# m96-chan/PyGPUkit

Measured on AMD Instinct MI355X. Metric: decode tokens/sec/GPU + prefill TFLOPS (% MFMA peak), Qwen3-0.6B bf16, higher is better.
Workload: dtype bf16

## Files before the change

pygpukit_amd/csrc/engine_attn.hip.h:

```cpp
#pragma once

#include "attn_core.hip.h"
#include "engine_state.hip.h"

namespace pgk {

struct AttnArgs {
    const float* qkv;
    int qkv_ld;
    const bf16 *q_gamma, *k_gamma;
    float eps;
    const float *rope_cos, *rope_sin;
    bf16 *kcache, *vcache;
    const int32_t* positions;
    int hq, hkv, max_seq;
    int span;
    float scale;
    float* part;
    int nsplit;
    float* attn_direct;
    const bf16* w_o;
    const bf16* w_o_scale;
    int H, rows_per_block;
    float* opart;
    bf16* attn_direct16;
    int g_total, g_off;
};

template <int D, int G>
struct NewToken {
    float qf[G][8], kn[8], vn[8];
    uint4 qb[G], kbits, vbits;
};

template <int G>
struct NewTokenRaw {
    float4 lo[G + 2], hi[G + 2];
    uint4 gq, gk;
    float4 cs[2], sn[2];
};

template <int D, int G>
__device__ __forceinline__ void new_token_load(const AttnArgs& a, int b, int kvh, int lane, NewTokenRaw<G>& r) {
    constexpr int LPR = D / 8, HALF = D / 2;
    const int sub = lane % LPR;
    const float* row = a.qkv + (size_t)b * a.qkv_ld;
#pragma unroll
    for (int g = 0; g < G + 2; ++g) {
        const unsigned eoff = (g < G) ? (unsigned)(kvh * a.g_total + a.g_off + g) * D : (g == G ? (unsigned)(a.hq + kvh) * D : (unsigned)(a.hq + a.hkv + kvh) * D);
        r.lo[g] = *reinterpret_cast<const float4*>(row + eoff + sub * 8);
        r.hi[g] = *reinterpret_cast<const float4*>(row + eoff + sub * 8 + 4);
    }
    r.gq = r.gk = make_uint4(0, 0, 0, 0);
    if (a.q_gamma != nullptr) {
        r.gq = *reinterpret_cast<const uint4*>(a.q_gamma + sub * 8);
        r.gk = *reinterpret_cast<const uint4*>(a.k_gamma + sub * 8);
    }
    const int dd = (sub * 8) % HALF;
    const float* cs = a.rope_cos + (size_t)b * HALF + dd;
    const float* sn = a.rope_sin + (size_t)b * HALF + dd;
    r.cs[0] = *reinterpret_cast<const float4*>(cs); r.cs[1] = *reinterpret_cast<const float4*>(cs + 4);
    r.sn[0] = *reinterpret_cast<const float4*>(sn); r.sn[1] = *reinterpret_cast<const float4*>(sn + 4);
}

template <int D, int G>
__device__ __forceinline__ void new_token_finish(const AttnArgs& a, int lane, const NewTokenRaw<G>& r, NewToken<D, G>& t) {
    constexpr int LPR = D / 8;
    const int sub = lane % LPR;
    float raw[G + 2][8], gq[8], gk[8];
#pragma unroll
    for (int g = 0; g < G + 2; ++g) {
        raw[g][0] = r.lo[g].x; raw[g][1] = r.lo[g].y; raw[g][2] = r.lo[g].z; raw[g][3] = r.lo[g].w;
        raw[g][4] = r.hi[g].x; raw[g][5] = r.hi[g].y; raw[g][6] = r.hi[g].z; raw[g][7] = r.hi[g].w;
    }
    const bool has_norm = a.q_gamma != nullptr;
    if (has_norm) {
        WTraits<bf16>::decode(r.gq, gq);
        WTraits<bf16>::decode(r.gk, gk);
    } else {
#pragma unroll
        for (int j = 0; j < 8; ++j) gq[j] = gk[j] = 1.f;
    }
    const float csv[8] = {r.cs[0].x, r.cs[0].y, r.cs[0].z, r.cs[0].w, r.cs[1].x, r.cs[1].y, r.cs[1].z, r.cs[1].w};
    const float snv[8] = {r.sn[0].x, r.sn[0].y, r.sn[0].z, r.sn[0].w, r.sn[1].x, r.sn[1].y, r.sn[1].z, r.sn[1].w};
    auto norm_rope = [&](const float (&xin)[8], const float (&gamma)[8], float (&o)[8]) {
        float x[8];
#pragma unroll
        for (int j = 0; j < 8; ++j) x[j] = xin[j];
        if (has_norm) {
            float ss = 0.f;
#pragma unroll
            for (int j = 0; j < 8; ++j) ss = fmaf(x[j], x[j], ss);
            ss = group_sum<LPR>(ss);
            const float inv = 1.0f / sqrtf(ss / D + a.eps);
#pragma unroll
            for (int j = 0; j < 8; ++j) x[j] = x[j] * inv * gamma[j];
        }
        const bool lo = sub < LPR / 2;
#pragma unroll
        for (int j = 0; j < 8; ++j) {
            const float other = xor_half<LPR>(x[j]);
            o[j] = lo ? (x[j] * csv[j] - other * snv[j]) : (x[j] * csv[j] + other * snv[j]);
        }
    };
#pragma unroll
    for (int g = 0; g < G; ++g) {
        norm_rope(raw[g], gq, t.qf[g]);
#pragma unroll
        for (int j = 0; j < 8; ++j) t.qf[g][j] *= a.scale;
        Vec<bf16> qv;
        qv.from_float(t.qf[g]);
        qv.to_float(t.qf[g]);
        t.qb[g] = qv.raw;
    }
    norm_rope(raw[G], gk, t.kn);
#pragma unroll
    for (int j = 0; j < 8; ++j) t.vn[j] = raw[G + 1][j];
    Vec<bf16> kb, vb;
    kb.from_float(t.kn);
    vb.from_float(t.vn);
    kb.to_float(t.kn);
    vb.to_float(t.vn);
    t.kbits = kb.raw;
    t.vbits = vb.raw;
}

template <int D, int G>
__device__ __forceinline__ void prepare_new_token(const AttnArgs& a, int b, int kvh, int pos, int lane, NewToken<D, G>& t) {
    NewTokenRaw<G> r;
    new_token_load<D, G>(a, b, kvh, lane, r);
    new_token_finish<D, G>(a, lane, r, t);
}

template <int D, int G>
__device__ __forceinline__ void fold_new_token(const NewToken<D, G>& t, DecodeState<G>& st) {
    constexpr int LPR = D / 8;
    float s[G];
#pragma unroll
    for (int g = 0; g < G; ++g) {
        float dsum = 0.f;
#pragma unroll
        for (int j = 0; j < 8; ++j) dsum = fmaf(t.qf[g][j], t.kn[j], dsum);
        dsum = group_sum<LPR>(dsum);
        s[g] = dsum;
    }
    st.update(s, t.vn);
}

template <int D, int G, bool DIRECT>
__global__ __launch_bounds__(256) void attn_decode_kernel(unsigned long long* tl, AttnArgs a) {
    const TLStamp tls(tl);
    constexpr int LPR = D / 8, PPW = 64 / LPR, RS = D + 2;
    __shared__ __attribute__((aligned(16))) float lds[4 * PPW * G * RS];
    __shared__ float attn_out[DIRECT ? G * D : 1];
    const int lane = threadIdx.x & 63, wid = threadIdx.x >> 6, sub = lane % LPR;
    const int kvh = blockIdx.y, b = blockIdx.z;
    const size_t head_off = (((size_t)b * a.hkv + kvh) * a.max_seq) * D;
    if constexpr (DIRECT) {
        constexpr int U0 = 8, UB = 4;
        NewTokenRaw<G> raw;
        new_token_load<D, G>(a, b, kvh, lane, raw);
        __builtin_amdgcn_sched_barrier(0);
        KVBatch<U0> kb0;
        kv_issue<D, U0, 4>(kb0, a.kcache + head_off, a.vcache + head_off, wid * PPW, a.max_seq - 1, lane);
        __builtin_amdgcn_sched_barrier(0);
        const int pos = load_uniform_i32(a.positions + b);
        const int c1 = min(pos, a.max_seq);
        KVBatch<UB> kb1;
        kv_issue<D, UB, 4>(kb1, a.kcache + head_off, a.vcache + head_off, U0 * 4 * PPW + wid * PPW, max(c1 - 1, 0), lane);
        __builtin_amdgcn_sched_barrier(0);
        NewToken<D, G> t;
        new_token_finish<D, G>(a, lane, raw, t);
        if (pos < a.max_seq && wid == 0 && lane < LPR && a.g_off == 0) {
            *reinterpret_cast<uint4*>(a.kcache + head_off + (size_t)pos * D + sub * 8) = t.kbits;
            *reinterpret_cast<uint4*>(a.vcache + head_off + (size_t)pos * D + sub * 8) = t.vbits;
        }
        DecodeState<G> st;
        st.init();
        kv_consume<D, G, U0, 4>(kb0, wid * PPW, c1, t.qb, lane, st);
        kv_consume<D, G, UB, 4>(kb1, U0 * 4 * PPW + wid * PPW, c1, t.qb, lane, st);
        if (c1 > (U0 + UB) * 4 * PPW) decode_walk_trips<D, G>(a.kcache + head_off, a.vcache + head_off, (U0 + UB) * 4 * PPW, c1, t.qb, lane, wid, st);
        if (pos < a.max_seq && wid == 0 && lane < LPR) fold_new_token<D, G>(t, st);
        decode_block_merge_lds<D, G>(st, lds, attn_out, lane, wid);
        if (a.attn_direct16) {
            for (int e = threadIdx.x; e < G * D; e += 256) a.attn_direct16[((size_t)b * a.hq + (size_t)kvh * a.g_total + a.g_off) * D + e] = from_f<bf16>(attn_out[e]);
        } else {
            for (int e = threadIdx.x; e < G * D; e += 256) a.attn_direct[((size_t)b * a.hq + (size_t)kvh * a.g_total + a.g_off) * D + e] = attn_out[e];
        }
        tls.end();
        return;
    }
    constexpr int U1 = 8;
    const int chunk = decode_chunk_len(a.span, a.nsplit, 4 * PPW);
    const int c0 = (int)blockIdx.x * chunk;
    NewTokenRaw<G> raw;
    new_token_load<D, G>(a, b, kvh, lane, raw);
    __builtin_amdgcn_sched_barrier(0);
    KVBatch<U1> kb0;
    kv_issue<D, U1, 4>(kb0, a.kcache + head_off, a.vcache + head_off, c0 + wid * PPW, a.max_seq - 1, lane);
    __builtin_amdgcn_sched_barrier(0);
    const int pos = load_uniform_i32(a.positions + b);
    const int ctx = min(pos + 1, a.max_seq);
    tls.phase(0);
    NewToken<D, G> t;
    new_token_finish<D, G>(a, lane, raw, t);
    tls.phase(1);
    const bool last_slice = (int)blockIdx.x == a.nsplit - 1;
    const int c1 = last_slice ? ctx : min(c0 + chunk, ctx);
    const bool owns_new = (pos < a.max_seq) && (pos >= c0) && (last_slice || pos < c0 + chunk);
    if (owns_new && wid == 0 && lane < LPR && a.g_off == 0) {
        *reinterpret_cast<uint4*>(a.kcache + head_off + (size_t)pos * D + sub * 8) = t.kbits;
        *reinterpret_cast<uint4*>(a.vcache + head_off + (size_t)pos * D + sub * 8) = t.vbits;
    }
    DecodeState<G> st;
    st.init();
    const int cend = owns_new ? min(c1, pos) : c1;
    kv_consume<D, G, U1, 4>(kb0, c0 + wid * PPW, cend, t.qb, lane, st);
    if (cend > c0 + U1 * 4 * PPW)
        decode_walk_trips<D, G>(a.kcache + head_off, a.vcache + head_off, c0 + U1 * 4 * PPW, cend, t.qb, lane, wid, st);
    if (owns_new && wid == 0 && lane < LPR) fold_new_token<D, G>(t, st);
    tls.phase(2);
    if constexpr (DIRECT) {
        decode_block_merge_lds<D, G>(st, lds, attn_out, lane, wid);
        for (int e = threadIdx.x; e < G * D; e += 256) a.attn_direct[((size_t)b * a.hq + (size_t)kvh * a.g_total + a.g_off) * D + e] = attn_out[e];
    } else {
        decode_block_merge<D, G>(st, lds, a.part + (((size_t)b * a.hq + (size_t)kvh * a.g_total + a.g_off) * a.nsplit + blockIdx.x) * RS,
                                 (size_t)a.nsplit * RS, lane, wid);
    }
    tls.end();
}

template <int D>
__global__ void attn_merge_kernel(unsigned long long* tl, const float* part, float* attn, int hq, int nsplit) {
    const TLStamp tls(tl);
    __shared__ float w_s[64];
    __shared__ float inv_l;
    const int h = blockIdx.x, b = blockIdx.y, d = threadIdx.x;
    const float* recs = part + ((size_t)b * hq + h) * nsplit * (D + 2);
    if (threadIdx.x < 64) {
        const int s = threadIdx.x;
        const int sc = min(s, nsplit - 1);
        float m = recs[(size_t)sc * (D + 2)], l = recs[(size_t)sc * (D + 2) + 1];
        if (s >= nsplit) { m = -INFINITY; l = 0.f; }
        const float mx = wave_max(m);
        const float w = (m == -INFINITY) ? 0.f : __expf(m - mx);
        const float tot = wave_sum(w * l);
        w_s[s] = w;
        if (s == 0) inv_l = tot > 0.f ? 1.0f / tot : 0.f;
    }
    __syncthreads();
    float o = 0.f;
    int s = 0;
    for (; s + 8 <= nsplit; s += 8) {
        float v[8];
#pragma unroll
        for (int u = 0; u < 8; ++u) v[u] = recs[(size_t)(s + u) * (D + 2) + 2 + d];
#pragma unroll
        for (int u = 0; u < 8; ++u) o = fmaf(w_s[s + u], v[u], o);
    }
    for (; s < nsplit; ++s) o = fmaf(w_s[s], recs[(size_t)s * (D + 2) + 2 + d], o);
    attn[((size_t)b * hq + h) * D + d] = o * inv_l;
    tls.end();
}

template <int D, int G>
__global__ __launch_bounds__(256) void attn_oproj_kernel(unsigned long long* tl, AttnArgs a) {
    const TLStamp tls(tl);
#ifdef PGK_PHASE_STAMPS
    if (threadIdx.x == 0) g_phase_tl = tl;
    __syncthreads();
#endif
    constexpr int NWV = 4;
    constexpr int LPR = D / 8, PPW = 64 / LPR, RS = D + 2;
    constexpr int GD = G * D, LPW = GD / 8;
    constexpr int RPP = NWV * 64 / LPW;
    constexpr int PRE = 4;
    constexpr int U0 = 12;
    __shared__ __attribute__((aligned(16))) float lds[NWV * PPW * G * RS];
    __shared__ __attribute__((aligned(16))) float attn[GD];
    const int lane = threadIdx.x & 63, wid = __builtin_amdgcn_readfirstlane(threadIdx.x >> 6), sub = lane % LPR;
    const int kvh = blockIdx.x % a.hkv, rb = blockIdx.x / a.hkv, b = blockIdx.z;
    const int r0 = rb * a.rows_per_block;
    const int lr = threadIdx.x % LPW, rip = threadIdx.x / LPW;
    const int npass = a.rows_per_block / RPP;
    const bf16* wbase = a.w_o + (size_t)kvh * GD + lr * 8;
    const int ldw = a.hq * D;
    const size_t head_off = (((size_t)b * a.hkv + kvh) * a.max_seq) * D;
    uint4 pre[PRE];
    KVBatch<U0> kb0;
    NewTokenRaw<G> raw;
    new_token_load<D, G>(a, b, kvh, lane, raw);
    __builtin_amdgcn_sched_barrier(0);
    kv_issue<D, U0, NWV>(kb0, a.kcache + head_off, a.vcache + head_off, wid * PPW, a.max_seq - 1, lane);
#pragma unroll
    for (int p = 0; p < PRE; ++p)
        pre[p] = load_nt16(wbase + (size_t)(r0 + min(p, npass - 1) * RPP + rip) * ldw);
    __builtin_amdgcn_sched_barrier(0);
    const int pos = load_uniform_i32(a.positions + b);
    tls.phase(0);
    NewToken<D, G> t;
    new_token_finish<D, G>(a, lane, raw, t);
    if (rb == 0 && pos < a.max_seq && wid == 0 && lane < LPR) {
        *reinterpret_cast<uint4*>(a.kcache + head_off + (size_t)pos * D + sub * 8) = t.kbits;
        *reinterpret_cast<uint4*>(a.vcache + head_off + (size_t)pos * D + sub * 8) = t.vbits;
    }
    tls.phase(1);
    DecodeState<G> st;
    st.init();
    const int c1 = min(pos, a.max_seq);
    kv_consume<D, G, U0, NWV>(kb0, wid * PPW, c1, t.qb, lane, st);
    if (c1 > U0 * NWV * PPW)
        decode_walk_trips<D, G, 8, NWV>(a.kcache + head_off, a.vcache + head_off, U0 * NWV * PPW, c1, t.qb, lane, wid, st);
    if (wid == 0 && lane < LPR) fold_new_token<D, G>(t, st);
    tls.phase(2);
    decode_block_merge_lds<D, G, NWV>(st, lds, attn, lane, wid);
    tls.phase(3);

    float xf[8];
    {
        const float4 u = *reinterpret_cast<const float4*>(attn + lr * 8), v = *reinterpret_cast<const float4*>(attn + lr * 8 + 4);
        xf[0] = u.x; xf[1] = u.y; xf[2] = u.z; xf[3] = u.w; xf[4] = v.x; xf[5] = v.y; xf[6] = v.z; xf[7] = v.w;
    }
    float* outp = a.opart + ((size_t)b * a.hkv + kvh) * a.H;
    for (int p = 0; p < npass; ++p) {
        const int row = r0 + p * RPP + rip;
        uint4 w = (p < PRE) ? pre[p < PRE ? p : 0] : load_nt16(wbase + (size_t)row * ldw);
        float wf[8];
        WTraits<bf16>::decode(w, wf);
        float acc = 0.f;
#pragma unroll
        for (int j = 0; j < 8; ++j) acc = fmaf(wf[j], xf[j], acc);
        acc = group_sum<LPW>(acc);
        if (lr == 0) outp[row] = acc;
    }
    tls.phase(4);
    tls.end();
}

constexpr int AM_CHUNK = 192;

__device__ __forceinline__ int am_koff(int row, int ch) { return row * 256 + ((ch ^ (row & 15)) << 4); }
__device__ __forceinline__ int am_voff(int row, int ch) { return row * 256 + ((ch ^ (((row & 3) << 2) | ((row >> 2) & 3))) << 4); }

template <int G, bool OPROJ = true>
__global__ __launch_bounds__(256) void attn_oproj_mfma_kernel(unsigned long long* tl, AttnArgs a) {
    const TLStamp tls(tl);
    typedef __bf16 am_bf16x8 __attribute__((ext_vector_type(8)));
    typedef float am_f32x4 __attribute__((ext_vector_type(4)));
    typedef short am_v4s __attribute__((ext_vector_type(4)));
    constexpr int D = 128, NWV = 4, LPR = 16, RS = D + 4;
    constexpr int GD = G * D, LPW = GD / 8, RPP = NWV * 64 / LPW, PRE = OPROJ ? 4 : 0;
    extern __shared__ __attribute__((aligned(16))) char am_lds[];
    char* k_lds = am_lds;
    char* v_lds = am_lds + AM_CHUNK * 256;
    __shared__ __attribute__((aligned(16))) float part[NWV + 1][G][RS];
    __shared__ __attribute__((aligned(16))) float attn[GD];
    const int lane = threadIdx.x & 63, wid = __builtin_amdgcn_readfirstlane(threadIdx.x >> 6);
    const int l15 = lane & 15, q4 = lane >> 4;
    const int kvh = blockIdx.x % a.hkv, rb = blockIdx.x / a.hkv, b = blockIdx.z;
    const int r0 = rb * a.rows_per_block;
    const int lr = threadIdx.x % LPW, rip = threadIdx.x / LPW;
    const int npass = a.rows_per_block / RPP;
    const bf16* wbase = a.w_o + (size_t)kvh * GD + lr * 8;
    const int ldw = a.hq * D;
    const size_t head_off = (((size_t)b * a.hkv + kvh) * a.max_seq) * D;
    const bf16* kc = a.kcache + head_off;
    const bf16* vc = a.vcache + head_off;

    auto dma = [](const void* src, uint32_t lds_addr) {
        asm volatile("s_mov_b32 m0, %1\n\ts_nop 0\n\tglobal_load_lds_dwordx4 %0, off" ::"v"(src), "s"(lds_addr) : "memory", "m0");
    };
    auto lds_u32 = [](const void* p) { return (uint32_t)(uintptr_t)(__attribute__((address_space(3))) const char*)p; };
    constexpr int HB = (G + 2) * 512;
    constexpr int NRAW = (HB + 1024 + 1023) / 1024;
    __shared__ __attribute__((aligned(16))) char raw_lds[NWV][NRAW * 1024];
    {
        const char* row = reinterpret_cast<const char*>(a.qkv + (size_t)b * a.qkv_ld);
        const char* cosr = reinterpret_cast<const char*>(a.rope_cos + (size_t)b * 64);
        const char* sinr = reinterpret_cast<const char*>(a.rope_sin + (size_t)b * 64);
        const char* gqp = a.q_gamma ? reinterpret_cast<const char*>(a.q_gamma) : cosr;
        const char* gkp = a.k_gamma ? reinterpret_cast<const char*>(a.k_gamma) : cosr;
#pragma unroll
        for (int i = 0; i < NRAW; ++i) {
            const int o = 1024 * i + 16 * lane;
            const char* src;
            if (o < HB) {
                const int hs = o >> 9, within = o & 511;
                const int elem = (hs < G) ? (kvh * a.g_total + a.g_off + hs) * D : (hs == G ? (a.hq + kvh) * D : (a.hq + a.hkv + kvh) * D);
                src = row + (size_t)elem * 4 + within;
            } else {
                const int o2 = min(o - HB, 1023), seg = o2 >> 8, within = o2 & 255;
                src = (seg == 0 ? gqp : seg == 1 ? gkp : seg == 2 ? cosr : sinr) + within;
            }
            dma(src, lds_u32(&raw_lds[wid][0]) + 1024 * i);
        }
    }
    auto stage = [&](int c0) {
#pragma unroll
        for (int i = 0; i < AM_CHUNK / 4 / NWV; ++i) {
            const int j = wid + NWV * i;
            const int rl = 4 * j + q4, rg = min(c0 + rl, a.max_seq - 1);
            dma(kc + (size_t)rg * D + ((l15 ^ (rl & 15)) << 3), lds_u32(k_lds) + j * 1024);
        }
#pragma unroll
        for (int i = 0; i < AM_CHUNK / 4 / NWV; ++i) {
            const int j = wid + NWV * i;
            const int rl = 4 * j + q4, rg = min(c0 + rl, a.max_seq - 1);
            dma(vc + (size_t)rg * D + ((l15 ^ (((rl & 3) << 2) | ((rl >> 2) & 3))) << 3), lds_u32(v_lds) + j * 1024);
        }
    };
    stage(0);
    uint4 pre[PRE > 0 ? PRE : 1];
#pragma unroll
    for (int p = 0; p < PRE; ++p) pre[p] = load_nt16(wbase + (size_t)(r0 + min(p, npass - 1) * RPP + rip) * ldw);
    __builtin_amdgcn_sched_barrier(0);
    const int pos = load_uniform_i32(a.positions + b);
    tls.phase(0);
    asm volatile("s_waitcnt vmcnt(%0)" ::"n"(2 * (AM_CHUNK / 4 / NWV) + PRE) : "memory");
    __shared__ __attribute__((aligned(16))) uint4 q_sh[G][16], k_sh[16], v_sh[16];
    {
        const char* slot = &raw_lds[wid][0];
        const int sub = l15;
        const int dd = (sub * 8) % 64;
        float csv[8], snv[8];
        {
            const float4 c0v = *reinterpret_cast<const float4*>(slot + HB + 512 + dd * 4), c1v = *reinterpret_cast<const float4*>(slot + HB + 512 + dd * 4 + 16);
            const float4 s0v = *reinterpret_cast<const float4*>(slot + HB + 768 + dd * 4), s1v = *reinterpret_cast<const float4*>(slot + HB + 768 + dd * 4 + 16);
            csv[0] = c0v.x; csv[1] = c0v.y; csv[2] = c0v.z; csv[3] = c0v.w; csv[4] = c1v.x; csv[5] = c1v.y; csv[6] = c1v.z; csv[7] = c1v.w;
            snv[0] = s0v.x; snv[1] = s0v.y; snv[2] = s0v.z; snv[3] = s0v.w; snv[4] = s1v.x; snv[5] = s1v.y; snv[6] = s1v.z; snv[7] = s1v.w;
        }
        const bool has_norm = a.q_gamma != nullptr;
        for (int item = wid; item < G + 2; item += NWV) {
            const float4 lo = *reinterpret_cast<const float4*>(slot + item * 512 + sub * 32), hi = *reinterpret_cast<const float4*>(slot + item * 512 + sub * 32 + 16);
            float x[8] = {lo.x, lo.y, lo.z, lo.w, hi.x, hi.y, hi.z, hi.w};
            if (item < G + 1) {
                if (has_norm) {
                    float gm[8];
                    WTraits<bf16>::decode(*reinterpret_cast<const uint4*>(slot + HB + (item < G ? 0 : 256) + sub * 16), gm);
                    float ss = 0.f;
#pragma unroll
                    for (int j = 0; j < 8; ++j) ss = fmaf(x[j], x[j], ss);
                    ss = group_sum<LPR>(ss);
                    const float inv = 1.0f / sqrtf(ss / D + a.eps);
#pragma unroll
                    for (int j = 0; j < 8; ++j) x[j] = x[j] * inv * gm[j];
                }
                const bool lo_half = sub < LPR / 2;
                float o8[8];
#pragma unroll
                for (int j = 0; j < 8; ++j) {
                    const float other = xor_half<LPR>(x[j]);
                    o8[j] = lo_half ? (x[j] * csv[j] - other * snv[j]) : (x[j] * csv[j] + other * snv[j]);
                }
#pragma unroll
                for (int j = 0; j < 8; ++j) x[j] = (item < G) ? o8[j] * a.scale : o8[j];
            }
            Vec<bf16> vb;
            vb.from_float(x);
            if (lane < 16) {
                if (item < G) q_sh[item][lane] = vb.raw;
                else if (item == G) k_sh[lane] = vb.raw;
                else v_sh[lane] = vb.raw;
            }
        }
    }
    tls.phase(1);
    uint4 qf[4];
    const int c1 = min(pos, a.max_seq);
    float m_run = -INFINITY, l_run = 0.f;
    am_f32x4 o[D / 16];
#pragma unroll
    for (int i = 0; i < D / 16; ++i) o[i] = am_f32x4{0.f, 0.f, 0.f, 0.f};
    const int tq = l15 >> 2, tp = l15 & 3;
    for (int c0 = 0; c0 == 0 || c0 < c1; c0 += AM_CHUNK) {
        if (c0 > 0) {
            __syncthreads();
            stage(c0);
        }
        if (c0 > 0) asm volatile("s_waitcnt vmcnt(0)" ::: "memory");
        else asm volatile("s_waitcnt vmcnt(%0)" ::"n"(PRE) : "memory");
        __syncthreads();
        if (c0 == 0) {
#pragma unroll
            for (int ks = 0; ks < 4; ++ks) {
                const uint4 v = q_sh[min(l15, G - 1)][4 * ks + q4];
                qf[ks] = l15 < G ? v : make_uint4(0, 0, 0, 0);
            }
            if (wid == NWV - 1 && lane < LPR) {
                float kn[8], vn[8];
                Vec<bf16> kb, vb2;
                kb.raw = k_sh[lane]; vb2.raw = v_sh[lane];
                kb.to_float(kn); vb2.to_float(vn);
                const bool live = pos < a.max_seq;
#pragma unroll
                for (int g = 0; g < G; ++g) {
                    Vec<bf16> qb;
                    qb.raw = q_sh[g][lane];
                    float qv[8];
                    qb.to_float(qv);
                    float dsum = 0.f;
#pragma unroll
                    for (int j = 0; j < 8; ++j) dsum = fmaf(qv[j], kn[j], dsum);
                    dsum = group_sum<LPR>(dsum);
                    if (lane == 0) { part[NWV][g][D] = live ? dsum : -INFINITY; part[NWV][g][D + 1] = live ? 1.f : 0.f; }
#pragma unroll
                    for (int j = 0; j < 8; ++j) part[NWV][g][lane * 8 + j] = vn[j];
                }
                if (rb == 0 && live) {
                    *reinterpret_cast<uint4*>(a.kcache + head_off + (size_t)pos * D + lane * 8) = kb.raw;
                    *reinterpret_cast<uint4*>(a.vcache + head_off + (size_t)pos * D + lane * 8) = vb2.raw;
                }
            }
        }
        am_f32x4 s[3];
        float mx = -INFINITY;
#pragma unroll
        for (int u = 0; u < 3; ++u) {
            const int tile = wid + NWV * u;
            s[u] = am_f32x4{0.f, 0.f, 0.f, 0.f};
            if (c0 + 16 * tile < c1) {
#pragma unroll
                for (int ks = 0; ks < 4; ++ks) {
                    const uint4 ka = *reinterpret_cast<const uint4*>(k_lds + am_koff(16 * tile + l15, 4 * ks + q4));
                    s[u] = __builtin_amdgcn_mfma_f32_16x16x32_bf16(__builtin_bit_cast(am_bf16x8, ka), __builtin_bit_cast(am_bf16x8, qf[ks]), s[u], 0, 0, 0);
                }
            }
#pragma unroll
            for (int r = 0; r < 4; ++r) {
                const bool ok = c0 + 16 * tile + 4 * q4 + r < c1;
                s[u][r] = ok ? s[u][r] : -INFINITY;
                mx = fmaxf(mx, s[u][r]);
            }
        }
        mx = fmaxf(mx, __shfl_xor(mx, 16, 64));
        mx = fmaxf(mx, __shfl_xor(mx, 32, 64));
        const float m_new = fmaxf(m_run, mx);
        const float alpha = (m_new == -INFINITY) ? 1.f : __expf(m_run - m_new);
        float ls = 0.f;
        uint32_t pk[3][2];
#pragma unroll
        for (int u = 0; u < 3; ++u) {
            float p[4];
#pragma unroll
            for (int r = 0; r < 4; ++r) p[r] = (m_new == -INFINITY) ? 0.f : __expf(s[u][r] - m_new);
            pk[u][0] = pack_bf16x2(p[0], p[1]);
            pk[u][1] = pack_bf16x2(p[2], p[3]);
            ls += (__uint_as_float(pk[u][0] << 16) + __uint_as_float(pk[u][0] & 0xFFFF0000u)) + (__uint_as_float(pk[u][1] << 16) + __uint_as_float(pk[u][1] & 0xFFFF0000u));
        }
        ls += __shfl_xor(ls, 16, 64);
        ls += __shfl_xor(ls, 32, 64);
        l_run = l_run * alpha + ls;
        m_run = m_new;
#pragma unroll
        for (int i = 0; i < D / 16; ++i)
#pragma unroll
            for (int r = 0; r < 4; ++r) o[i][r] *= alpha;
#pragma unroll
        for (int st2 = 0; st2 < 2; ++st2) {
            const int ta = wid + NWV * (2 * st2), tb = (st2 == 0) ? wid + NWV : ta;
            if (c0 + 16 * ta < c1) {
                const uint4 pf = make_uint4(pk[2 * st2][0], pk[2 * st2][1], st2 == 0 ? pk[1][0] : 0u, st2 == 0 ? pk[1][1] : 0u);
                const int ra = 16 * ta + 4 * q4 + tq, rbv = 16 * tb + 4 * q4 + tq;
#pragma unroll
                for (int i = 0; i < D / 16; ++i) {
                    const am_v4s a0 = __builtin_amdgcn_ds_read_tr16_b64_v4i16((__attribute__((address_space(3))) am_v4s*)(v_lds + am_voff(ra, 2 * i + (tp >> 1)) + 8 * (tp & 1)));
                    const am_v4s a1 = __builtin_amdgcn_ds_read_tr16_b64_v4i16((__attribute__((address_space(3))) am_v4s*)(v_lds + am_voff(rbv, 2 * i + (tp >> 1)) + 8 * (tp & 1)));
                    const uint2 u0 = __builtin_bit_cast(uint2, a0), u1 = __builtin_bit_cast(uint2, a1);
                    const uint4 va = make_uint4(u0.x, u0.y, u1.x, u1.y);
                    o[i] = __builtin_amdgcn_mfma_f32_16x16x32_bf16(__builtin_bit_cast(am_bf16x8, va), __builtin_bit_cast(am_bf16x8, pf), o[i], 0, 0, 0);
                }
            }
        }
    }
    tls.phase(2);
    if (l15 < G) {
        if (q4 == 0) { part[wid][l15][D] = m_run; part[wid][l15][D + 1] = l_run; }
#pragma unroll
        for (int i = 0; i < D / 16; ++i)
            *reinterpret_cast<float4*>(&part[wid][l15][16 * i + 4 * q4]) = make_float4(o[i][0], o[i][1], o[i][2], o[i][3]);
    }
    __syncthreads();
    for (int e = threadIdx.x; e < GD; e += 256) {
        const int g = e / D, d = e % D;
        float mstar = -INFINITY;
#pragma unroll
        for (int w = 0; w <= NWV; ++w) mstar = fmaxf(mstar, part[w][g][D]);
        float num = 0.f, den = 0.f;
#pragma unroll
        for (int w = 0; w <= NWV; ++w) {
            const float mw = part[w][g][D];
            const float wgt = (mw == -INFINITY) ? 0.f : __expf(mw - mstar);
            num = fmaf(wgt, part[w][g][d], num);
            den = fmaf(wgt, part[w][g][D + 1], den);
        }
        attn[e] = den > 0.f ? num / den : 0.f;
    }
    __syncthreads();
    tls.phase(3);
    if constexpr (OPROJ) {
        float xf[8];
        {
            const float4 u = *reinterpret_cast<const float4*>(attn + lr * 8), v = *reinterpret_cast<const float4*>(attn + lr * 8 + 4);
            xf[0] = u.x; xf[1] = u.y; xf[2] = u.z; xf[3] = u.w; xf[4] = v.x; xf[5] = v.y; xf[6] = v.z; xf[7] = v.w;
        }
        float* outp = a.opart + ((size_t)b * a.hkv + kvh) * a.H;
        auto wo_fixed = [&](auto np_c) {
            constexpr int NP = decltype(np_c)::value;
            static_assert(NP <= PRE, "every pass of a fixed count is preloaded");
            float acc[NP];
#pragma unroll
            for (int p = 0; p < NP; ++p) {
                float wf[8];
                WTraits<bf16>::decode(pre[p], wf);
                acc[p] = 0.f;
#pragma unroll
                for (int j = 0; j < 8; ++j) acc[p] = fmaf(wf[j], xf[j], acc[p]);
            }
#pragma unroll
            for (int p = 0; p < NP; ++p) acc[p] = group_sum<LPW>(acc[p]);
            if (lr == 0) {
#pragma unroll
                for (int p = 0; p < NP; ++p) outp[r0 + p * RPP + rip] = acc[p];
            }
        };
        if (npass == 4) wo_fixed(std::integral_constant<int, 4>{});
        else if (npass == 2) wo_fixed(std::integral_constant<int, 2>{});
        else if (npass == 1) wo_fixed(std::integral_constant<int, 1>{});
        else {
            for (int p = 0; p < npass; ++p) {
                const int row = r0 + p * RPP + rip;
                uint4 w = (p < PRE) ? pre[p < PRE ? p : 0] : load_nt16(wbase + (size_t)row * ldw);
                float wf[8];
                WTraits<bf16>::decode(w, wf);
                float acc = 0.f;
#pragma unroll
                for (int j = 0; j < 8; ++j) acc = fmaf(wf[j], xf[j], acc);
                acc = group_sum<LPW>(acc);
                if (lr == 0) outp[row] = acc;
            }
        }
    } else {
        const size_t ob = ((size_t)b * a.hq + (size_t)kvh * G) * D;
        if (a.attn_direct16) {
            for (int e = threadIdx.x; e < GD; e += 256) a.attn_direct16[ob + e] = from_f<bf16>(attn[e]);
        } else {
            for (int e = threadIdx.x; e < GD; e += 256) a.attn_direct[ob + e] = attn[e];
        }
    }
    tls.phase(4);
    tls.end();
}

template <int D, int G, bool FP8>
__global__ __launch_bounds__(256) void attn_merge_oproj_kernel(unsigned long long* tl, AttnArgs a) {
    const TLStamp tls(tl);
    constexpr int RS = D + 2, GD = G * D;
    constexpr int NWT = FP8 ? 16 : 8;
    constexpr int LPW = GD / NWT;
    constexpr int RPP = 256 / LPW;
    constexpr int PRE = 4;
    static_assert(LPW <= 64 && 256 % LPW == 0, "row slice must fit a wave");
    __shared__ float w_s[G][64];
    __shared__ float inv_l[G];
    __shared__ __attribute__((aligned(16))) float attn[GD];
    const int lane = threadIdx.x & 63, wid = __builtin_amdgcn_readfirstlane(threadIdx.x >> 6);
    const int kvh = blockIdx.x % a.hkv, rb = blockIdx.x / a.hkv, b = blockIdx.z;
    const int r0 = rb * a.rows_per_block;
    const int lr = threadIdx.x % LPW, rip = threadIdx.x / LPW;
    const int npass = a.rows_per_block / RPP;
    const int ldw = a.hq * D;
    const int col0 = kvh * GD + lr * NWT;
    const char* wbase = reinterpret_cast<const char*>(a.w_o) + (size_t)col0 * (FP8 ? 1 : 2);
    const size_t row_bytes = (size_t)ldw * (FP8 ? 1 : 2);
    const float* hrecs = a.part + ((size_t)b * a.hq + (size_t)kvh * G) * a.nsplit * RS;
    float m = -INFINITY, l = 0.f;
    if (wid < G) {
        const int sc = min(lane, a.nsplit - 1);
        m = hrecs[((size_t)wid * a.nsplit + sc) * RS];
        l = hrecs[((size_t)wid * a.nsplit + sc) * RS + 1];
    }
    constexpr int EPT = (GD + 255) / 256, RPRE = 32;
    float rv[EPT][RPRE];
#pragma unroll
    for (int i = 0; i < EPT; ++i) {
        const int e = min((int)threadIdx.x + 256 * i, GD - 1), g = e / D, d = e % D;
        const float* recs = hrecs + (size_t)g * a.nsplit * RS + 2 + d;
#pragma unroll
        for (int u = 0; u < RPRE; ++u) rv[i][u] = recs[(size_t)min(u, a.nsplit - 1) * RS];
    }
    __builtin_amdgcn_sched_barrier(0);
    uint4 pre[PRE];
    float psc[PRE];
#pragma unroll
    for (int p = 0; p < PRE; ++p) {
        const int row = r0 + min(p, npass - 1) * RPP + rip;
        pre[p] = load_nt16(wbase + (size_t)row * row_bytes);
        if constexpr (FP8) psc[p] = to_f(a.w_o_scale[(size_t)(row >> 7) * (ldw >> 7) + (col0 >> 7)]);
    }
    __builtin_amdgcn_sched_barrier(0);
    tls.phase(0);
    if (wid < G) {
        if (lane >= a.nsplit) { m = -INFINITY; l = 0.f; }
        const float mx = wave_max(m);
        const float w = (m == -INFINITY) ? 0.f : __expf(m - mx);
        const float tot = wave_sum(w * l);
        w_s[wid][lane] = w;
        if (lane == 0) inv_l[wid] = tot > 0.f ? 1.0f / tot : 0.f;
    }
    __syncthreads();
    tls.phase(1);
#pragma unroll
    for (int i = 0; i < EPT; ++i) {
        const int e = (int)threadIdx.x + 256 * i;
        if (e < GD) {
            const int g = e / D, d = e % D;
            const float* recs = hrecs + (size_t)g * a.nsplit * RS;
            float o = 0.f;
#pragma unroll
            for (int u = 0; u < RPRE; ++u) o = fmaf(u < a.nsplit ? w_s[g][u] : 0.f, rv[i][u], o);
            for (int s2 = RPRE; s2 < a.nsplit; ++s2) o = fmaf(w_s[g][s2], recs[(size_t)s2 * RS + 2 + d], o);
            attn[e] = o * inv_l[g];
        }
    }
    __syncthreads();
    tls.phase(2);
    float xf[NWT];
#pragma unroll
    for (int i = 0; i < NWT / 4; ++i) {
        const float4 u = *reinterpret_cast<const float4*>(attn + lr * NWT + 4 * i);
        xf[4 * i] = u.x; xf[4 * i + 1] = u.y; xf[4 * i + 2] = u.z; xf[4 * i + 3] = u.w;
    }
    float* outp = a.opart + ((size_t)b * a.hkv + kvh) * a.H;
    for (int p = 0; p < npass; ++p) {
        const int row = r0 + p * RPP + rip;
        uint4 w;
        float sc = 1.f;
        if (p < PRE) {
            w = pre[p < PRE ? p : 0];
            if constexpr (FP8) sc = psc[p < PRE ? p : 0];
        } else {
            w = load_nt16(wbase + (size_t)row * row_bytes);
            if constexpr (FP8) sc = to_f(a.w_o_scale[(size_t)(row >> 7) * (ldw >> 7) + (col0 >> 7)]);
        }
        float wf[NWT];
        if constexpr (FP8) WTraits<fp8e4m3>::decode(w, wf);
        else WTraits<bf16>::decode(w, wf);
        float acc = 0.f;
#pragma unroll
        for (int j = 0; j < NWT; ++j) acc = fmaf(wf[j], xf[j], acc);
        acc = group_sum<LPW>(acc * sc);
        if (lr == 0) outp[row] = acc;
    }
    tls.end();
}

template <int G, bool OPROJ = true>
static hipError_t launch_attn_mfma(dim3 grid, hipStream_t st, const AttnArgs& a) {
    constexpr int lds = 2 * AM_CHUNK * 256;
    static bool attr = false;
    if (!attr) {
        const hipError_t he = hipFuncSetAttribute(reinterpret_cast<const void*>(&attn_oproj_mfma_kernel<G, OPROJ>), hipFuncAttributeMaxDynamicSharedMemorySize, lds);
        if (he != hipSuccess) return he;
        attr = true;
    }
    return launch_k(attn_oproj_mfma_kernel<G, OPROJ>, grid, dim3(256), lds, st, a);
}

template <class F>
static hipError_t with_group(int G, F f) {
    return G == 1 ? f(std::integral_constant<int, 1>{}) : G == 2 ? f(std::integral_constant<int, 2>{}) : G == 4 ? f(std::integral_constant<int, 4>{}) : hipSuccess;
}

template <int D, int G>
static hipError_t launch_attn_decode(bool direct, dim3 grid, hipStream_t st, const AttnArgs& a) {
    return direct ? launch_k(attn_decode_kernel<D, G, true>, grid, dim3(256), 0, st, a) : launch_k(attn_decode_kernel<D, G, false>, grid, dim3(256), 0, st, a);
}

enum AttnKernel { AK_FUSED_MFMA = 0, AK_FUSED_DOT2, AK_DIRECT_MFMA, AK_DIRECT, AK_SPLIT };
enum AttnTail { AT_NONE = 0, AT_MERGE, AT_MERGE_OPROJ_BF16, AT_MERGE_OPROJ_FP8 };
struct AttnChoice { AttnKernel kernel; AttnTail tail; int nsplit, span; bool out_bf16; };
inline AttnChoice attn_choice(const Engine* e, int m, int step_span, const AttnFlags& f) {
    const auto& c = e->cfg;
    const int D = c.head_dim, G = c.num_heads / c.num_kv_heads;
    AttnChoice ch{};
    ch.span = (step_span > 0 && step_span < c.max_seq_len) ? step_span : c.max_seq_len;
    int ns = e->cu_count * (m >= 4 ? 2 : 1) / (c.num_kv_heads * m);
    const int ns_cap = ceil_div(ch.span, 64) < e->nsplit ? ceil_div(ch.span, 64) : e->nsplit;
    ns = ns < 1 ? 1 : (ns > ns_cap ? ns_cap : ns);
    ch.nsplit = f.direct ? 1 : ceil_div(ch.span, decode_chunk_len(ch.span, ns, 4 * (64 / (D / 8))));
    ch.out_bf16 = f.direct && f.direct_bf16;
    if (!group_instantiated(G)) ch.kernel = f.direct ? AK_DIRECT : AK_SPLIT;
    else if (f.fused) ch.kernel = (D == 128 && e->attn_mfma) ? AK_FUSED_MFMA : AK_FUSED_DOT2;
    else if (f.direct) ch.kernel = (D == 128 && e->attn_mfma && m * (int)c.num_kv_heads <= e->cu_count) ? AK_DIRECT_MFMA : AK_DIRECT;
    else ch.kernel = AK_SPLIT;
    const bool f8 = c.weight_format == 1 || c.weight_format == 2;
    ch.tail = f.merged ? (f8 ? AT_MERGE_OPROJ_FP8 : AT_MERGE_OPROJ_BF16) : ((!f.fused && !f.direct) ? AT_MERGE : AT_NONE);
    return ch;
}

template <int D>
static pgk_status launch_attn_d(const StepCtx& cx, int layer, const AttnFlags& af) {
    const bool fused = af.fused, direct = af.direct;
    Engine* e = cx.e;
    const int b0 = cx.b0, m = cx.M;
    const hipStream_t st = cx.st;
    const auto& c = e->cfg;
    const auto& L = e->layers[layer];
    const int G = c.num_heads / c.num_kv_heads;
    const size_t lofs = (size_t)layer * e->kv_layer_elems() + (size_t)b0 * c.num_kv_heads * c.max_seq_len * c.head_dim;
    AttnArgs a{};
    a.qkv = e->qkv + (size_t)b0 * e->qkv_dim();
    a.qkv_ld = e->qkv_dim();
    a.q_gamma = c.use_qk_norm ? (const bf16*)L.q_norm : nullptr;
    a.k_gamma = c.use_qk_norm ? (const bf16*)L.k_norm : nullptr;
    a.eps = c.norm_eps;
    a.rope_cos = e->cur_cos + (size_t)b0 * (D / 2); a.rope_sin = e->cur_sin + (size_t)b0 * (D / 2);
    a.kcache = e->kcache + lofs; a.vcache = e->vcache + lofs;
    a.positions = e->positions + b0;
    a.hq = c.num_heads; a.hkv = c.num_kv_heads; a.max_seq = c.max_seq_len;
    const AttnChoice pick = attn_choice(e, m, e->step_span, af);
    a.span = pick.span;
    a.scale = 1.0f / sqrtf((float)D);
    a.part = e->part + (size_t)b0 * c.num_heads * e->nsplit * (D + 2);
    a.nsplit = pick.nsplit;
    a.w_o = (const bf16*)L.w_o; a.w_o_scale = (const bf16*)L.s_o; a.H = c.hidden_size; a.rows_per_block = e->oproj_rows;
    a.opart = e->opart ? e->opart + (size_t)b0 * c.num_kv_heads * c.hidden_size : nullptr;
    if (direct) {
        a.attn_direct = e->attnv + (size_t)b0 * c.num_heads * D;
        if (pick.out_bf16) a.attn_direct16 = e->attnv16 + (size_t)b0 * c.num_heads * D;
    }
    dim3 grid = fused ? dim3((c.hidden_size / e->oproj_rows) * c.num_kv_heads, 1, m) : dim3(a.nsplit, c.num_kv_heads, m);
    hipError_t he = hipSuccess;
    a.g_total = G;
    a.g_off = 0;
    if (!group_instantiated(G)) {
        PGK_REQUIRE(!fused, "engine: fused attention needs a GQA group of 1, 2 or 4");
        for (int off = 0; off < G;) {
            const int gc = head_chunk(G, off);
            a.g_off = off;
            he = with_group(gc, [&](auto g) { return launch_attn_decode<D, decltype(g)::value>(direct, grid, st, a); });
            PGK_CHECK_HIP(he);
            ++*cx.launches;
            off += gc;
        }
    } else {
        he = with_group(G, [&](auto g) {
            constexpr int GG = decltype(g)::value;
            if constexpr (D == 128) {
                if (pick.kernel == AK_FUSED_MFMA) return launch_attn_mfma<GG>(grid, st, a);
                if (pick.kernel == AK_DIRECT_MFMA) return launch_attn_mfma<GG, false>(dim3(c.num_kv_heads, 1, m), st, a);
            }
            if (pick.kernel == AK_FUSED_DOT2) return launch_k(attn_oproj_kernel<D, GG>, grid, dim3(256), 0, st, a);
            return launch_attn_decode<D, GG>(pick.kernel == AK_DIRECT, grid, st, a);
        });
        PGK_CHECK_HIP(he);
        ++*cx.launches;
    }
    if (pick.tail == AT_MERGE_OPROJ_BF16 || pick.tail == AT_MERGE_OPROJ_FP8) {
        PGK_REQUIRE(!fused && !direct && group_instantiated(G), "engine: merged o_proj on an unsupported attention path");
        mark(KC_OPROJ);
        a.rows_per_block = e->moproj_rows;
        const dim3 g2((c.hidden_size / e->moproj_rows) * c.num_kv_heads, 1, m);
        PGK_REQUIRE(c.weight_format != 3, "engine: merged o_proj has no NVF4 form");
        const bool f8 = pick.tail == AT_MERGE_OPROJ_FP8;
        he = with_group(G, [&](auto g) {
            constexpr int GG = decltype(g)::value;
            return f8 ? launch_k(attn_merge_oproj_kernel<D, GG, true>, g2, dim3(256), 0, st, a) : launch_k(attn_merge_oproj_kernel<D, GG, false>, g2, dim3(256), 0, st, a);
        });
        PGK_CHECK_HIP(he);
        ++*cx.launches;
    } else if (pick.tail == AT_MERGE) {
        PGK_CHECK_HIP(launch_k(attn_merge_kernel<D>, dim3(c.num_heads, m), dim3(D), 0, st, (const float*)a.part,
                               e->attnv + (size_t)b0 * c.num_heads * D, (int)c.num_heads, (int)a.nsplit));
        ++*cx.launches;
    }
    return PGK_OK;
}

static pgk_status launch_attn(const StepCtx& cx, int layer, const AttnFlags& af) {
    return cx.e->cfg.head_dim == 128 ? launch_attn_d<128>(cx, layer, af) : launch_attn_d<64>(cx, layer, af);
}

}
```

pygpukit_amd/csrc/engine_common.hip.h:

```cpp
#pragma once

#include <hip/hip_ext.h>

#include <tuple>
#include <vector>

#include "gemv_core.hip.h"
#include "pgk_internal.h"

namespace pgk {

enum { KC_EMBED = 0, KC_NORM_QKV, KC_ATTN, KC_OPROJ, KC_GATEUP, KC_DOWN, KC_LMHEAD, KC_ARGMAX, KC_COUNT };
constexpr int TL_MAXWG = 2048;

struct TLInfo { int cls, nwg; };
struct Probe {
    bool timing = false;
    int cur_cls = 0;
    std::vector<hipEvent_t> ev;
    std::vector<int> cls;
    size_t used = 0;
    unsigned long long* tl = nullptr;
    int tl_cap = 0;
    std::vector<TLInfo> info;
};
extern thread_local Probe* g_probe;

template <class... KArgs, class... Args>
inline hipError_t launch_k(void (*kernel)(KArgs...), dim3 grid, dim3 block, size_t lds, hipStream_t st, Args... args) {
    static_assert(sizeof...(KArgs) == sizeof...(Args) + 1, "launch_k: every decode-step kernel takes a leading timeline pointer");
    Probe* p = g_probe;
    unsigned long long* tl = nullptr;
    auto go = [&](hipEvent_t e0, hipEvent_t e1) {
        std::tuple<KArgs...> formal{tl, args...};
        std::apply([&](auto... ka) {
            if (e0) hipExtLaunchKernelGGL(kernel, grid, block, (uint32_t)lds, st, e0, e1, 0, ka...);
            else hipLaunchKernelGGL(kernel, grid, block, (uint32_t)lds, st, ka...);
        }, formal);
    };
    if (p) {
        const int nwg = (int)(grid.x * grid.y * grid.z);
        if (p->tl && (int)p->info.size() < p->tl_cap) tl = p->tl + (size_t)p->info.size() * TL_MAXWG * 2;
        p->info.push_back(TLInfo{p->cur_cls, nwg});
        if (p->timing) {
            if (2 * p->used + 1 >= p->ev.size()) {
                hipEvent_t e0, e1;
                if (hipEventCreate(&e0) != hipSuccess || hipEventCreate(&e1) != hipSuccess) return hipErrorOutOfMemory;
                p->ev.push_back(e0);
                p->ev.push_back(e1);
                p->cls.push_back(0);
            }
            p->cls[p->used] = p->cur_cls;
            go(p->ev[2 * p->used], p->ev[2 * p->used + 1]);
            ++p->used;
            return hipGetLastError();
        }
    }
    go(nullptr, nullptr);
    return hipGetLastError();
}
static inline void mark(int cls) { if (g_probe) g_probe->cur_cls = cls; }

struct TLStamp {
    unsigned long long* p;
    unsigned long long t0;
    __device__ __forceinline__ explicit TLStamp(unsigned long long* tl) : p(tl), t0(0) {
        if (p) t0 = __builtin_amdgcn_s_memrealtime();
    }
    __device__ __forceinline__ void phase(int i) const {
#ifdef PGK_PHASE_STAMPS
        if (p && threadIdx.x == 0) {
            const unsigned wg = blockIdx.x + gridDim.x * (blockIdx.y + gridDim.y * blockIdx.z);
            if (wg < 256u) p[2 * (256 + 4 * wg) + i] = __builtin_amdgcn_s_memrealtime();
        }
#endif
    }
    __device__ __forceinline__ void end() const {
        if (p) {
            __syncthreads();
            const unsigned wg = blockIdx.x + gridDim.x * (blockIdx.y + gridDim.y * blockIdx.z);
            if (threadIdx.x == 0 && wg < (unsigned)TL_MAXWG) {
                p[2 * wg] = t0;
                p[2 * wg + 1] = __builtin_amdgcn_s_memrealtime();
            }
        }
    }
};

enum { PRO_NORM = 0, PRO_PLAIN = 1, PRO_NORM_SUM = 3 };
enum { EPI_STORE = 0, EPI_RESID = 1, EPI_SWIGLU = 2, EPI_LOGITS = 3 };

struct FusedArgs {
    const void* w;
    const bf16* wscale;
    const bf16* wp;
    int N, K;
    const float* h;
    const bf16* gamma;
    float eps;
    const float* xin;
    const float* part;
    int nsplit;
    float* h_out;
    const float* res;
    float* out;
    int ld_out;
    float* amax_val;
    int* amax_idx;
    const bf16* xin16;
    bf16* out16;
};

pgk_status batched_proj(bool fp8, int pro, int epi, const FusedArgs& a, int M, hipStream_t st, int nblk_logits = 0);
pgk_status norm_rows_bf16(const float* h, const bf16* gamma, bf16* x16, int M, int K, float eps, hipStream_t st);

}
```

Measured before the change: 1701.

## Split K/V staging waits and hoist kernel args for attention-oproj MFMA kernel

Passes hot scalar arguments (qkv, kcache, rope tables, gammas, hkv, max_seq) directly as kernel parameters so they arrive in SGPRs early, and uses a 2D grid (kvh, rb) instead of a div/mod decode. K/V chunk staging now uses SGPR-base DMA with precomputed per-lane offsets and separate vmcnt waits for K and V, so QK^T can start before V has landed. The next chunk is issued without a leading barrier, and the KV-cache write of the new token moves to the end of the kernel on one wave. This adds host-side validation constraints (g_off==0, fixed qkv_ld) and tighter reliance on exact wait-count ordering. Dropping the barrier before restaging risks overwriting LDS that other waves may still be reading.

Result: faster. 1742 (median of 6 runs) (+2.4%).

```diff
diff --git a/pygpukit_amd/csrc/engine_attn.hip.h b/pygpukit_amd/csrc/engine_attn.hip.h
--- a/pygpukit_amd/csrc/engine_attn.hip.h
+++ b/pygpukit_amd/csrc/engine_attn.hip.h
@@ -343,8 +343,10 @@
 __device__ __forceinline__ int am_voff(int row, int ch) { return row * 256 + ((ch ^ (((row & 3) << 2) | ((row >> 2) & 3))) << 4); }
 
 template <int G, bool OPROJ = true>
-__global__ __launch_bounds__(256) void attn_oproj_mfma_kernel(unsigned long long* tl, AttnArgs a) {
-    const TLStamp tls(tl);
+__global__ __launch_bounds__(256) void attn_oproj_mfma_kernel(const float* qkv_, bf16* kcache_, const float* rope_cos_, const float* rope_sin_,
+                                                              const bf16* q_gamma_, const bf16* k_gamma_, int hkv_, int max_seq_,
+                                                              unsigned long long* tl, AttnArgs a) {
+    const TLStamp tls(tl, TLStamp::Deferred{});
     typedef __bf16 am_bf16x8 __attribute__((ext_vector_type(8)));
     typedef float am_f32x4 __attribute__((ext_vector_type(4)));
     typedef short am_v4s __attribute__((ext_vector_type(4)));
@@ -357,15 +359,11 @@
     __shared__ __attribute__((aligned(16))) float attn[GD];
     const int lane = threadIdx.x & 63, wid = __builtin_amdgcn_readfirstlane(threadIdx.x >> 6);
     const int l15 = lane & 15, q4 = lane >> 4;
-    const int kvh = blockIdx.x % a.hkv, rb = blockIdx.x / a.hkv, b = blockIdx.z;
-    const int r0 = rb * a.rows_per_block;
+    const int kvh = blockIdx.x, rb = blockIdx.y, b = blockIdx.z;
+    const int hq = G * hkv_;
     const int lr = threadIdx.x % LPW, rip = threadIdx.x / LPW;
-    const int npass = a.rows_per_block / RPP;
-    const bf16* wbase = a.w_o + (size_t)kvh * GD + lr * 8;
-    const int ldw = a.hq * D;
-    const size_t head_off = (((size_t)b * a.hkv + kvh) * a.max_seq) * D;
-    const bf16* kc = a.kcache + head_off;
-    const bf16* vc = a.vcache + head_off;
+    const size_t head_off = (((size_t)b * hkv_ + kvh) * max_seq_) * D;
+    const bf16* kc = kcache_ + head_off;
 
     auto dma = [](const void* src, uint32_t lds_addr) {
         asm volatile("s_mov_b32 m0, %1\n\ts_nop 0\n\tglobal_load_lds_dwordx4 %0, off" ::"v"(src), "s"(lds_addr) : "memory", "m0");
@@ -374,49 +372,82 @@
     constexpr int HB = (G + 2) * 512;
     constexpr int NRAW = (HB + 1024 + 1023) / 1024;
     __shared__ __attribute__((aligned(16))) char raw_lds[NWV][NRAW * 1024];
+    auto dma_s = [](const void* base, uint32_t voff, uint32_t lds_addr) {
+        asm volatile("s_mov_b32 m0, %2\n\ts_nop 0\n\tglobal_load_lds_dwordx4 %0, %1" ::"v"(voff), "s"(base), "s"(lds_addr) : "memory", "m0");
+    };
     {
-        const char* row = reinterpret_cast<const char*>(a.qkv + (size_t)b * a.qkv_ld);
-        const char* cosr = reinterpret_cast<const char*>(a.rope_cos + (size_t)b * 64);
-        const char* sinr = reinterpret_cast<const char*>(a.rope_sin + (size_t)b * 64);
-        const char* gqp = a.q_gamma ? reinterpret_cast<const char*>(a.q_gamma) : cosr;
-        const char* gkp = a.k_gamma ? reinterpret_cast<const char*>(a.k_gamma) : cosr;
+        const char* row = reinterpret_cast<const char*>(qkv_ + (size_t)b * ((hq + 2 * hkv_) * D));
+        const char* cosr = reinterpret_cast<const char*>(rope_cos_ + (size_t)b * 64);
+        const char* sinr = reinterpret_cast<const char*>(rope_sin_ + (size_t)b * 64);
+        const char* gqp = q_gamma_ ? reinterpret_cast<const char*>(q_gamma_) : cosr;
+        const char* gkp = k_gamma_ ? reinterpret_cast<const char*>(k_gamma_) : cosr;
+        auto head_byte = [&](int hs) { return (uint32_t)((hs < G) ? (kvh * G + hs) * D : (hs == G ? (hq + kvh) * D : (hq + hkv_ + kvh) * D)) * 4u; };
 #pragma unroll
         for (int i = 0; i < NRAW; ++i) {
             const int o = 1024 * i + 16 * lane;
-            const char* src;
-            if (o < HB) {
-                const int hs = o >> 9, within = o & 511;
-                const int elem = (hs < G) ? (kvh * a.g_total + a.g_off + hs) * D : (hs == G ? (a.hq + kvh) * D : (a.hq + a.hkv + kvh) * D);
-                src = row + (size_t)elem * 4 + within;
+            if (1024 * (i + 1) <= HB) {
+                const uint32_t within = (uint32_t)(16 * lane) & 511u;
+                dma_s(row, (lane < 32 ? head_byte(2 * i) : head_byte(2 * i + 1)) + within, lds_u32(&raw_lds[wid][0]) + 1024 * i);
             } else {
-                const int o2 = min(o - HB, 1023), seg = o2 >> 8, within = o2 & 255;
-                src = (seg == 0 ? gqp : seg == 1 ? gkp : seg == 2 ? cosr : sinr) + within;
-            }
-            dma(src, lds_u32(&raw_lds[wid][0]) + 1024 * i);
-        }
-    }
-    auto stage = [&](int c0) {
-#pragma unroll
-        for (int i = 0; i < AM_CHUNK / 4 / NWV; ++i) {
-            const int j = wid + NWV * i;
-            const int rl = 4 * j + q4, rg = min(c0 + rl, a.max_seq - 1);
-            dma(kc + (size_t)rg * D + ((l15 ^ (rl & 15)) << 3), lds_u32(k_lds) + j * 1024);
-        }
-#pragma unroll
-        for (int i = 0; i < AM_CHUNK / 4 / NWV; ++i) {
-            const int j = wid + NWV * i;
-            const int rl = 4 * j + q4, rg = min(c0 + rl, a.max_seq - 1);
-            dma(vc + (size_t)rg * D + ((l15 ^ (((rl & 3) << 2) | ((rl >> 2) & 3))) << 3), lds_u32(v_lds) + j * 1024);
+                const char* src;
+                if (o < HB) {
+                    src = row + head_byte(o >> 9) + (o & 511);
+                } else {
+                    const int o2 = min(o - HB, 1023), seg = o2 >> 8, within = o2 & 255;
+                    src = (seg == 0 ? gqp : seg == 1 ? gkp : seg == 2 ? cosr : sinr) + within;
+                }
+                dma(src, lds_u32(&raw_lds[wid][0]) + 1024 * i);
+            }
+        }
+    }
+    uint32_t koff[4], voff[4];
+    {
+        const uint32_t wq = ((threadIdx.x >> 6) << 12) | ((uint32_t)q4 << 8);
+#pragma unroll
+        for (int r = 0; r < 4; ++r) {
+            koff[r] = wq + 1024 * r + ((uint32_t)(l15 ^ (4 * r + q4)) << 4);
+            voff[r] = wq + 1024 * r + ((uint32_t)(l15 ^ (4 * q4 + r)) << 4);
+        }
+    }
+    static_assert(AM_CHUNK == 16 * 3 * NWV, "a chunk is three 16-row tiles per wave: 12 K and 12 V requests per wave");
+    constexpr int NREQ = AM_CHUNK / 4 / NWV;
+    auto stage_image = [&](const bf16* head, const uint32_t (&off)[4], uint32_t lds_img, int c0) {
+        const bf16* base = head + (size_t)c0 * D;
+        const uint32_t dst = lds_img + wid * 4096;
+        if (c0 + AM_CHUNK <= max_seq_) {
+#pragma unroll
+            for (int u = 0; u < 3; ++u)
+#pragma unroll
+                for (int r = 0; r < 4; ++r) dma_s(base + u * 64 * D, off[r], dst + u * 16384 + r * 1024);
+        } else {
+            const uint32_t last = (uint32_t)(max_seq_ - 1 - c0) << 8;
+#pragma unroll
+            for (int u = 0; u < 3; ++u)
+#pragma unroll
+                for (int r = 0; r < 4; ++r) dma_s(base, min(off[r] + 16384u * u, last | (off[r] & 0xF0u)), dst + u * 16384 + r * 1024);
         }
     };
-    stage(0);
+    stage_image(kc, koff, lds_u32(k_lds), 0);
+    __builtin_amdgcn_sched_barrier(0);
+    const int pos = *(const __attribute__((address_space(4))) int32_t*)(a.positions + b);
+    const bf16* vc = a.vcache + head_off;
+    stage_image(vc, voff, lds_u32(v_lds), 0);
+    const int r0 = rb * a.rows_per_block;
+    const int npass = a.rows_per_block / RPP;
+    const bf16* wbase = a.w_o + (size_t)kvh * GD + lr * 8;
+    const int ldw = hq * D;
     uint4 pre[PRE > 0 ? PRE : 1];
 #pragma unroll
     for (int p = 0; p < PRE; ++p) pre[p] = load_nt16(wbase + (size_t)(r0 + min(p, npass - 1) * RPP + rip) * ldw);
     __builtin_amdgcn_sched_barrier(0);
-    const int pos = load_uniform_i32(a.positions + b);
     tls.phase(0);
-    asm volatile("s_waitcnt vmcnt(%0)" ::"n"(2 * (AM_CHUNK / 4 / NWV) + PRE) : "memory");
+    constexpr int W_NEW = 2 * NREQ + PRE;
+    constexpr int W_K0 = NREQ + PRE;
+    constexpr int W_V0 = PRE;
+    constexpr int W_K = NREQ;
+    constexpr int W_V = 0;
+    static_assert(NREQ == 12 && W_NEW == 24 + PRE && W_K0 == 12 + PRE && W_V0 == PRE && W_K == 12, "wait counts follow the request order above");
+    asm volatile("s_waitcnt vmcnt(%0)" ::"n"(W_NEW) : "memory");
     __shared__ __attribute__((aligned(16))) uint4 q_sh[G][16], k_sh[16], v_sh[16];
     {
         const char* slot = &raw_lds[wid][0];
@@ -429,7 +460,7 @@
             csv[0] = c0v.x; csv[1] = c0v.y; csv[2] = c0v.z; csv[3] = c0v.w; csv[4] = c1v.x; csv[5] = c1v.y; csv[6] = c1v.z; csv[7] = c1v.w;
             snv[0] = s0v.x; snv[1] = s0v.y; snv[2] = s0v.z; snv[3] = s0v.w; snv[4] = s1v.x; snv[5] = s1v.y; snv[6] = s1v.z; snv[7] = s1v.w;
         }
-        const bool has_norm = a.q_gamma != nullptr;
+        const bool has_norm = q_gamma_ != nullptr;
         for (int item = wid; item < G + 2; item += NWV) {
             const float4 lo = *reinterpret_cast<const float4*>(slot + item * 512 + sub * 32), hi = *reinterpret_cast<const float4*>(slot + item * 512 + sub * 32 + 16);
             float x[8] = {lo.x, lo.y, lo.z, lo.w, hi.x, hi.y, hi.z, hi.w};
@@ -466,7 +497,7 @@
     }
     tls.phase(1);
     uint4 qf[4];
-    const int c1 = min(pos, a.max_seq);
+    const int c1 = min(pos, max_seq_);
     float m_run = -INFINITY, l_run = 0.f;
     am_f32x4 o[D / 16];
 #pragma unroll
@@ -474,12 +505,14 @@
     const int tq = l15 >> 2, tp = l15 & 3;
     for (int c0 = 0; c0 == 0 || c0 < c1; c0 += AM_CHUNK) {
         if (c0 > 0) {
+            stage_image(kc, koff, lds_u32(k_lds), c0);
+            stage_image(vc, voff, lds_u32(v_lds), c0);
+            asm volatile("s_waitcnt vmcnt(%0)" ::"n"(W_K) : "memory");
+        } else {
             __syncthreads();
-            stage(c0);
-        }
-        if (c0 > 0) asm volatile("s_waitcnt vmcnt(0)" ::: "memory");
-        else asm volatile("s_waitcnt vmcnt(%0)" ::"n"(PRE) : "memory");
-        __syncthreads();
+            asm volatile("s_waitcnt vmcnt(%0)" ::"n"(W_K0) : "memory");
+        }
+        __builtin_amdgcn_sched_barrier(0);
         if (c0 == 0) {
 #pragma unroll
             for (int ks = 0; ks < 4; ++ks) {
@@ -491,7 +524,7 @@
                 Vec<bf16> kb, vb2;
                 kb.raw = k_sh[lane]; vb2.raw = v_sh[lane];
                 kb.to_float(kn); vb2.to_float(vn);
-                const bool live = pos < a.max_seq;
+                const bool live = pos < max_seq_;
 #pragma unroll
                 for (int g = 0; g < G; ++g) {
                     Vec<bf16> qb;
@@ -506,10 +539,6 @@
 #pragma unroll
                     for (int j = 0; j < 8; ++j) part[NWV][g][lane * 8 + j] = vn[j];
                 }
-                if (rb == 0 && live) {
-                    *reinterpret_cast<uint4*>(a.kcache + head_off + (size_t)pos * D + lane * 8) = kb.raw;
-                    *reinterpret_cast<uint4*>(a.vcache + head_off + (size_t)pos * D + lane * 8) = vb2.raw;
-                }
             }
         }
         am_f32x4 s[3];
@@ -555,6 +584,9 @@
         for (int i = 0; i < D / 16; ++i)
 #pragma unroll
             for (int r = 0; r < 4; ++r) o[i][r] *= alpha;
+        if (c0 > 0) asm volatile("s_waitcnt vmcnt(%0)" ::"n"(W_V) : "memory");
+        else asm volatile("s_waitcnt vmcnt(%0)" ::"n"(W_V0) : "memory");
+        __builtin_amdgcn_sched_barrier(0);
 #pragma unroll
         for (int st2 = 0; st2 < 2; ++st2) {
             const int ta = wid + NWV * (2 * st2), tb = (st2 == 0) ? wid + NWV : ta;
@@ -573,6 +605,10 @@
         }
     }
     tls.phase(2);
+    if (rb == 0 && wid == NWV - 1 && lane < LPR && pos < max_seq_) {
+        *reinterpret_cast<uint4*>(kcache_ + head_off + (size_t)pos * D + lane * 8) = k_sh[lane];
+        *reinterpret_cast<uint4*>(a.vcache + head_off + (size_t)pos * D + lane * 8) = v_sh[lane];
+    }
     if (l15 < G) {
         if (q4 == 0) { part[wid][l15][D] = m_run; part[wid][l15][D + 1] = l_run; }
 #pragma unroll
@@ -763,7 +799,8 @@
         if (he != hipSuccess) return he;
         attr = true;
     }
-    return launch_k(attn_oproj_mfma_kernel<G, OPROJ>, grid, dim3(256), lds, st, a);
+    if (a.hq != G * a.hkv || a.g_total != G || a.g_off != 0 || a.qkv_ld != (a.hq + 2 * a.hkv) * 128) return hipErrorInvalidValue;
+    return launch_k<8>(attn_oproj_mfma_kernel<G, OPROJ>, grid, dim3(256), lds, st, a.qkv, a.kcache, a.rope_cos, a.rope_sin, a.q_gamma, a.k_gamma, a.hkv, a.max_seq, a);
 }
 
 template <class F>
@@ -847,7 +884,7 @@
         he = with_group(G, [&](auto g) {
             constexpr int GG = decltype(g)::value;
             if constexpr (D == 128) {
-                if (pick.kernel == AK_FUSED_MFMA) return launch_attn_mfma<GG>(grid, st, a);
+                if (pick.kernel == AK_FUSED_MFMA) return launch_attn_mfma<GG>(dim3(c.num_kv_heads, c.hidden_size / e->oproj_rows, m), st, a);
                 if (pick.kernel == AK_DIRECT_MFMA) return launch_attn_mfma<GG, false>(dim3(c.num_kv_heads, 1, m), st, a);
             }
             if (pick.kernel == AK_FUSED_DOT2) return launch_k(attn_oproj_kernel<D, GG>, grid, dim3(256), 0, st, a);
diff --git a/pygpukit_amd/csrc/engine_common.hip.h b/pygpukit_amd/csrc/engine_common.hip.h
--- a/pygpukit_amd/csrc/engine_common.hip.h
+++ b/pygpukit_amd/csrc/engine_common.hip.h
@@ -26,13 +26,19 @@
 };
 extern thread_local Probe* g_probe;
 
-template <class... KArgs, class... Args>
+template <class Tup, size_t... I, size_t... J>
+inline auto tl_splice(unsigned long long* tl, const Tup& t, std::index_sequence<I...>, std::index_sequence<J...>) {
+    return std::make_tuple(std::get<I>(t)..., tl, std::get<sizeof...(I) + J>(t)...);
+}
+
+template <int TL_AT = 0, class... KArgs, class... Args>
 inline hipError_t launch_k(void (*kernel)(KArgs...), dim3 grid, dim3 block, size_t lds, hipStream_t st, Args... args) {
-    static_assert(sizeof...(KArgs) == sizeof...(Args) + 1, "launch_k: every decode-step kernel takes a leading timeline pointer");
+    static_assert(sizeof...(KArgs) == sizeof...(Args) + 1, "launch_k: every decode-step kernel takes a timeline pointer (leading unless TL_AT says otherwise)");
+    static_assert(TL_AT >= 0 && TL_AT <= (int)sizeof...(Args), "launch_k: timeline pointer position");
     Probe* p = g_probe;
     unsigned long long* tl = nullptr;
     auto go = [&](hipEvent_t e0, hipEvent_t e1) {
-        std::tuple<KArgs...> formal{tl, args...};
+        std::tuple<KArgs...> formal{tl_splice(tl, std::make_tuple(args...), std::make_index_sequence<TL_AT>{}, std::make_index_sequence<sizeof...(Args) - TL_AT>{})};
         std::apply([&](auto... ka) {
             if (e0) hipExtLaunchKernelGGL(kernel, grid, block, (uint32_t)lds, st, e0, e1, 0, ka...);
             else hipLaunchKernelGGL(kernel, grid, block, (uint32_t)lds, st, ka...);
@@ -67,6 +73,8 @@
     __device__ __forceinline__ explicit TLStamp(unsigned long long* tl) : p(tl), t0(0) {
         if (p) t0 = __builtin_amdgcn_s_memrealtime();
     }
+    struct Deferred {};
+    __device__ __forceinline__ TLStamp(unsigned long long* tl, Deferred) : p(tl), t0(__builtin_amdgcn_s_memrealtime()) {}
     __device__ __forceinline__ void phase(int i) const {
 #ifdef PGK_PHASE_STAMPS
         if (p && threadIdx.x == 0) {
```
